# AnthonyYates/FluidFramework

Hardware: AMD Instinct MI355X
Metric: sequenced ops applied/sec (whole node) + achieved HBM GB/s, 256k docs (higher is better)
Workload: dtype int32

## Files before the change

fluidframework_amd/csrc/reg_engine.hpp:

```cpp
#pragma once
#include <stddef.h>
#include <stdint.h>
#include <string.h>

#include "engine_types.hpp"
#include "reg_rows.hpp"
#include "wave_simd.hpp"

namespace mte {

constexpr u32 RG_LEVELS = 8;
constexpr u32 RG_HEAP = 511;
constexpr u32 RSEQ_LIVE = 0x7FFFFFFFu;
constexpr u32 RCL_LIVE = 0xFFu;
constexpr i32 REG_HANDOFF = 101;
constexpr u32 NS_SHIFT = 24, NS_MASK = 3u << NS_SHIFT;

enum RgProf : u32 {
    RP_TOTAL, RP_FETCH, RP_APPLY, RP_RESOLVE, RP_INSERT_SLOT, RP_SPLIT, RP_RANGE, RP_ZAMBONI, RP_SCOUR,
    RP_HEAP, RP_FIND_SEG, RP_PACK, RP_LRU, RP_OPS, RP_N_RESOLVE, RP_N_SCOUR, RP_N_SCOUR_CHANGED,
    RP_N_PACK, RP_N_POP, RP_N_SPLIT_BLK, RP_N_MOVE, RP_SPLIT_AT, RP_INS, RP_REM, RP_MSN, RP_ZAM_EDIT,
    RP_PACK_SIBS,
    RP_PACK_FUSED,
    RP_N
};
#if defined(MTE_PROFILE) && !defined(MTE_CPU)
#ifdef RG_PROF_ONLY
#define RG_ON(slot) ((slot) == RG_PROF_ONLY || (slot) == RP_TOTAL)
#else
#define RG_ON(slot) true
#endif
template <bool ON>
struct RgScope {
    u64& acc;
    u64 t0;
    __device__ __forceinline__ RgScope(u64& a) : acc(a), t0(ON ? __builtin_amdgcn_s_memtime() : 0) {}
    __device__ __forceinline__ ~RgScope() {
        if (ON) acc += __builtin_amdgcn_s_memtime() - t0;
    }
};
#define RG_PROF(slot) RgScope<RG_ON(slot)> _rg_scope_##slot(pf[slot])
#define RG_COUNT(slot, n) (pf[slot] += (u64)(n))
#elif defined(MTE_MARKERS) && !defined(MTE_CPU)
template <u32 S>
struct RgMark {
    __device__ __forceinline__ RgMark() { asm volatile("; MTE_BEGIN %0" ::"i"(S + 100)); }
    __device__ __forceinline__ ~RgMark() { asm volatile("; MTE_END %0" ::"i"(S + 100)); }
};
#define RG_PROF(slot) RgMark<slot> _rg_mark_##slot
#define RG_COUNT(slot, n) \
    do {                  \
    } while (0)
#else
#define RG_PROF(slot) \
    do {              \
    } while (0)
#define RG_COUNT(slot, n) \
    do {                  \
    } while (0)
#endif

#if defined(MTE_CPU) && defined(MTE_CPU_STATS)
enum RgStat : u32 {
    RS_OPS, RS_RESOLVE, RS_RES_ROWS, RS_RES_NROWS, RS_POP, RS_POP_BIG, RS_POP_HEAP, RS_FIND_ROWS, RS_SCOUR,
    RS_SCOUR_NOP, RS_SCOUR_SERIAL, RS_SCOUR_COPY, RS_PACK, RS_SPLIT_BLK, RS_MOVE_SLOTS, RS_SPLIT_AT,
    RS_ZAM_CALLS, RS_ZAM_POPS, RS_LRU_PUSH, RS_RANGE_ROWS, RS_DUO_HANDOVER, RS_DUO_SPEC_OK, RS_DUO_SPEC_REDO,
    RS_DUO_NO_RESOLVE, RS_DUO_W_ROWS,
    RS_REM, RS_REM_SAMEROW, RS_REM_SAMEROW_NOSPLIT, RS_RES2_ROWS, RS_PACK_SCOUR, RS_PACK_SCOUR_NOP,
    RS_PACK_SELF_CHANGED, RS_PACK_SIB_CHANGED, RS_PACK_ONE_ROW, RS_PACK_TWO_ROWS, RS_PACK_SERIAL, RS_PACK_GC,
    RS_PACK_CASCADE, RS_PACK_M8, RS_PACK_GROWS, RS_PACK_M_SUM, RS_PACK_KK_SUM,
    RS_LRU_REWRITE, RS_LRU_FOLDED,
    RS_PACK_FUSED, RS_PACK_FUSED_FB_SERIAL, RS_PACK_FUSED_FB_GC,
    RS_HIT_FIRST, RS_HIT_SECOND, RS_SPLIT_NEXT_ROW, RS_HEAP_REG1, RS_HEAP_REG2, RS_SIFT_SERIAL, RS_PACK_KK1, RS_PACK_KK2,
    RS_PACK_KK3, RS_PACK_KK4, RS_PACK_KK5, RS_PACK_KK6, RS_PACK_KK7, RS_PACK_REM, RS_PACK_INTERNAL, RS_ROOM_REFUSED, RS_N
};
inline u64 g_rg_stats[RS_N + 64];
#define RG_STAT(i, n) (g_rg_stats[i] += (u64)(n))
struct RgDuoStat {
    u64 w;
    bool popped, packed, pending;
    void settle_begin() {
        if (pending) RG_STAT(RS_DUO_NO_RESOLVE, 1);
        w = 0;
        popped = packed = pending = false;
    }
    void settle_end() {
        if (!popped) return;
        RG_STAT(RS_DUO_HANDOVER, 1);
        RG_STAT(RS_DUO_W_ROWS, __builtin_popcountll(w));
        pending = true;
    }
    void resolved(bool ok, u32 row) {
        if (!pending) return;
        pending = false;
        const u64 scanned = ok && row < 63 ? (2ull << row) - 1 : ~0ull;
        if (packed || (w & scanned)) RG_STAT(RS_DUO_SPEC_REDO, 1);
        else RG_STAT(RS_DUO_SPEC_OK, 1);
    }
};
inline RgDuoStat g_rg_duo;
#define RG_DUO(stmt) (g_rg_duo.stmt)
#else
#define RG_STAT(i, n) \
    do {              \
    } while (0)
#define RG_DUO(stmt) \
    do {             \
    } while (0)
#endif

#ifndef MTE_FUSED_PACK
#define MTE_FUSED_PACK 1
#endif
#ifndef MTE_STATE_REGS
#define MTE_STATE_REGS 5
#endif

struct RSeg {
    u32 len;
    i32 seq;
    u32 rseq;
    u32 meta;
    u32 toff;
    u32 cap;
    u32 rm;
    u32 sid;
    u32 props = 0;
    u32 rm2 = 0;
};
struct RFound {
    bool ok;
    u32 k;
    u32 cnt;
    i32 slot;
    i32 r;
    u32 row;
    u32 carry;
};

template <int NR = (int)RG_ROWS, bool PAGED = false, bool PROPS = false, bool WIDE = false>
struct RegEngine {
    static constexpr bool kProps = PROPS, kWide = WIDE;
    static constexpr bool kFoldLru = !PAGED && NR == (int)RG_ROWS;
    static constexpr bool kFusedPack = MTE_FUSED_PACK == 2 || (MTE_FUSED_PACK == 1 && !PAGED && NR == (int)RG_ROWS);
    static constexpr bool kOwnRows = !PAGED && NR == (int)RG_ROWS && !PROPS && !WIDE;
    static constexpr bool kHeapInPlace = kOwnRows && (MTE_STATE_REGS & 1) != 0;
    static constexpr bool kMulDiv = kOwnRows && (MTE_STATE_REGS & 4) != 0;
    static constexpr u32 MAXC = WIDE ? 64u : 32u;
    typedef simd::V V;
    typedef simd::B B;
    static constexpr u32 NBLK = (u32)NR * 8;
    typedef RowStore<NR, PAGED, PROPS, WIDE> Rows;
    typedef typename Rows::Row Row;

    simd::VA<RG_LEVELS> LV;
    struct HeapRegs {
        V r0, r1, x2, x3, x4, x5, x6, x7;
        SD V get(u32 i) const {
            switch (i) {
                case 0: return r0;
                case 1: return r1;
                case 2: return x2;
                case 3: return x3;
                case 4: return x4;
                case 5: return x5;
                case 6: return x6;
                default: return x7;
            }
        }
        SD void set(u32 i, V v) {
            switch (i) {
                case 0: r0 = v; break;
                case 1: r1 = v; break;
                case 2: x2 = v; break;
                case 3: x3 = v; break;
                case 4: x4 = v; break;
                case 5: x5 = v; break;
                case 6: x6 = v; break;
                default: x7 = v; break;
            }
        }
        SD void zero() { r0 = r1 = x2 = x3 = x4 = x5 = x6 = x7 = simd::splat(0); }
    };
    HeapRegs HK, HS;
    u32 n_lb, height, heapSize, segNext, arenaTop, arenaSel;
    i32 minSeq, curSeq, heapTop, status, failSeq;
    u32 n_gc, max_lb;
    u32 n_ops, n_msgs;
    SD u32 ops_n() const { return n_ops; }
    SD u32 msgs_n() const { return n_msgs; }
    SD void set_counts(u32 o, u32 m) {
        n_ops = o;
        n_msgs = m;
    }
    SD void count_op() { n_ops++; }
    SD void count_msg() { n_msgs++; }
    u32 lb_lim;
    bool adirty;
#if defined(MTE_PROFILE) && !defined(MTE_CPU)
    u64 pf[RP_N];
#endif
    const Params& p;
    u32 doc;
    u16* payload;
    u16* arena0;
    u32 seg_cap, arena_cap, payload_len;
    Rows rows;
#ifdef MTE_CPU
    u32& pool_rows = rows.at.pool_rows;
#endif
    SD void release_rows() { rows.release_rows(); }

    SD V ld_len(u32 r) const { return rows.ldf(r, 0, 0); }
    SD V ld_meta(u32 r) const { return rows.ldf(r, 0, 3); }
    SD V ld_sid(u32 r) const { return rows.ldf(r, 1, 3); }
    SD bool ensure_blocks(u32 nb) {
        if constexpr (PAGED) {
            if (rows.grow_rows((nb + 7) >> 3)) return true;
            fail(REG_HANDOFF, curSeq);
        } else {
            if (nb <= NBLK) return true;
            fail(MTE_DOC_CAPACITY, curSeq);
        }
        return false;
    }

    SD RegEngine(const Params& p_, u32 doc_, const RowsLds& g = RowsLds::solo_lean())
        : p(p_), doc(doc_), rows(g), res_mode(g.mode) {
        setup();
    }
// ... 186 lines not shown
        f.slot = -1;
        f.r = 0;
        f.row = 0;
        f.carry = 0;
        const u32 nrows = (n_lb + 7) >> 3;
        RG_STAT(RS_RESOLVE, 1);
        RG_STAT(RS_RES_NROWS, nrows);
        u32 carry = carry0;
        const B end = (L() & 7u) == 7u;
        auto hit_row = [&](const Row& w, u32 r, u64 hit, const V& v, const V& incl) MTE_LI {
            const u32 g = (u32)__builtin_ctzll(hit) >> 3;
            const u32 k = r * 8 + g, gb = g * 8;
            const V rr = (u32)pos - (incl - v);
            const B valid = w.len != 0u;
            const B seen = simd::sle(w.rseq, R) & (w.rseq != 0u);
            const B cand = in_group(k) & valid & (simd::slt(rr, v) | ((rr == 0u) & (v == 0u) & ~seen));
            const u64 cm = simd::ballot(cand);
            f.ok = true;
            f.k = k;
            f.cnt = (u32)__builtin_popcount(group_bits(simd::ballot(valid), k));
            f.row = r;
            f.carry = carry;
            rows.cache(r, w);
            if (cm) {
                const u32 l = (u32)__builtin_ctzll(cm);
                f.slot = (i32)(l - gb);
                f.r = (i32)simd::readlane(rr, l);
            }
        };
        const u32 last = nrows - 1;
        Row a = rows.row(r0), b;
        V v, incl;
        u64 hit = 0;
        bool inb = false;
        u32 r = r0;
        for (;;) {
            b = rows.ldrow(r + 1 < last ? r + 1 : last);
            RG_COUNT(RP_N_RESOLVE, 1);
            v = vis(a, R, C);
            RG_STAT(RS_RES_ROWS, 1);
            incl = simd::scan_incl(v) + carry;
            hit = simd::ballot(end & simd::sge(incl, pos));
            if (hit) break;
            carry = simd::readlane(incl, 63);
            if (++r >= nrows) break;
            a = rows.ldrow(r + 1 < last ? r + 1 : last);
            RG_COUNT(RP_N_RESOLVE, 1);
            v = vis(b, R, C);
            RG_STAT(RS_RES_ROWS, 1);
            incl = simd::scan_incl(v) + carry;
            hit = simd::ballot(end & simd::sge(incl, pos));
            if (hit) {
                inb = true;
                break;
            }
            carry = simd::readlane(incl, 63);
            if (++r >= nrows) break;
        }
        if (!hit) {
            RG_DUO(resolved(false, 0));
            return f;
        }
        RG_STAT(inb ? RS_HIT_SECOND : RS_HIT_FIRST, nrows >= 3);
        if (inb) a = b;
        hit_row(a, r, hit, v, incl);
        RG_DUO(resolved(true, f.row));
        return f;
    }

    SD u32 parent_of(u32 lv, u32 c, u32& first) const {
        const V cnt = LV.get(lv);
        const V incl = simd::scan_incl(cnt);
        const u64 m = simd::ballot(incl > c);
        const u32 pi = m ? (u32)__builtin_ctzll(m) : 0u;
        first = simd::readlane(incl, pi) - simd::readlane(cnt, pi);
        return pi;
    }
    SD void insert_after(u32 c, u32 lv) {
        for (u32 guard = 0; guard <= RG_LEVELS; guard++) {
            if (lv + 1 >= height) {
                if (lv >= RG_LEVELS) break;
                LV.set(lv, simd::sel(L() == 0u, 2u, simd::splat(0)));
                height++;
                return;
            }
            u32 first;
            const u32 pi = parent_of(lv, c, first);
            V P = LV.get(lv);
            const u32 nc = simd::readlane(P, pi) + 1;
            if (nc < 8) {
                LV.set(lv, simd::writelane(P, pi, nc));
                return;
            }
            P = simd::sel(L() > pi, simd::wave_shr1(P), P);
            P = simd::sel((L() == pi) | (L() == pi + 1), 4u, P);
            LV.set(lv, P);
            c = pi;
            lv++;
        }
        fail(MTE_DOC_CAPACITY, curSeq);
    }

    SD void shift_blocks(u32 from, i32 d) {
        if (d == 0) return;
        RG_COUNT(RP_N_MOVE, n_lb - from);
        const u32 n = (n_lb - from) * 8;
        RG_STAT(RS_MOVE_SLOTS, n);
        if (d > 0) {
            rows.mv_slots((from + (u32)d) * 8, from * 8, n);
        } else {
            rows.mv_slots((from - (u32)(-d)) * 8, from * 8, n);
            rows.zero_slots((n_lb - (u32)(-d)) * 8, (u32)(-d) * 8);
        }
    }

    bool lruFolded = false;
    SD u32 insert_slot(u32 k, u32 cnt, u32 j, const RSeg& rec, bool upd, u32 ul, u32 uc, i32 lru = 0) {
        RG_PROF(RP_INSERT_SLOT);
        lruFolded = false;
        if (cnt >= 8 || j > cnt) {
            fail(MTE_DOC_CAPACITY, curSeq);
            return NONE;
        }
        const u32 r = k >> 3, gb = gbase(k);
        Row& w = rows.rowref(r);
        const V sl = L() & 7u;
        const B ing = in_group(k);
        const B mv = ing & (sl > j);
        const B at = L() == gb + j;
        u32 ns = (simd::readlane(w.meta, gb) >> NS_SHIFT) & 3u;
        bool push = false;
        if constexpr (kFoldLru) {
            if (lru && cnt + 1 < 8) {
                lruFolded = true;
                if (ns != SC_TRUE && lru > curSeq) {
                    push = true;
                    ns = SC_TRUE;
                    ns_put(w, k, SC_TRUE);
                }
            }
        }
        if (upd) {
            const B lf = L() == gb + j - 1;
            w.len = simd::sel(lf, ul, w.len);
            w.cap = simd::sel(lf, uc, w.cap);
        }
        auto put = [&](V& x, u32 val) MTE_LI {
            x = simd::sel(mv, simd::row_shr1(x), x);
            x = simd::sel(at, val, x);
        };
        put(w.len, rec.len);
        put(w.seq, (u32)rec.seq);
        put(w.rseq, rec.rseq);
        put(w.meta, (rec.meta & ~NS_MASK) | (ns << NS_SHIFT));
        put(w.toff, rec.toff);
        put(w.cap, rec.cap);
        put(w.rm, rec.rm);
        put(w.sid, rec.sid);
        if constexpr (PROPS) put(w.props, rec.props);
        if constexpr (WIDE) put(w.rm2, rec.rm2);
        rows.writeback(r);
        if (push) {
            RG_STAT(RS_LRU_FOLDED, 1);
            heap_push(rec.sid, lru);
        }
        if (cnt + 1 < 8) return k;
        split_block(k);
        return j < 4 ? k : k + 1;
    }
    SD void split_block(u32 k) {
        RG_PROF(RP_SPLIT);
        RG_COUNT(RP_N_SPLIT_BLK, 1);
        RG_STAT(RS_SPLIT_BLK, 1);
        if (!ensure_blocks(n_lb + 1)) return;
        shift_blocks(k + 1, 1);
        const u32 r = k >> 3, r2 = (k + 1) >> 3;
        RG_STAT(RS_SPLIT_NEXT_ROW, r2 != r);
        const V sl = L() & 7u;
        const B lo = in_group(k + 1) & (sl < 4u), hi2 = in_group(k + 1) & (sl >= 4u), hi = in_group(k) & (sl >= 4u);
        const V src = (L() + (r2 == r ? 0u : 64u) - 4u) & 63u;
        Row w = rows.row(r);
        const u32 nsk = simd::readlane(w.meta, gbase(k)) & NS_MASK;
        Row w2 = r2 == r ? w : rows.ldrow(r2);
        auto mv = [&](V& x, V& y, u32 keepHi) MTE_LI {
            const V moved = simd::bperm(x, src);
            if (r2 == r) {
                x = simd::sel(lo, moved, x);
                x = simd::sel(hi2, 0u, x);
                x = simd::sel(hi, keepHi, x);
            } else {
                y = simd::sel(lo, moved, simd::sel(hi2, 0u, y));
                x = simd::sel(hi, keepHi, x);
            }
        };
        mv(w.len, w2.len, 0u);
        mv(w.seq, w2.seq, 0u);
        mv(w.rseq, w2.rseq, 0u);
        mv(w.meta, w2.meta, nsk);
        mv(w.toff, w2.toff, 0u);
        mv(w.cap, w2.cap, 0u);
        mv(w.rm, w2.rm, 0u);
        mv(w.sid, w2.sid, 0u);
        if constexpr (PROPS) mv(w.props, w2.props, 0u);
        if constexpr (WIDE) mv(w.rm2, w2.rm2, 0u);
        if (r2 == r) {
            w.meta = simd::sel(in_group(k + 1), w.meta & ~NS_MASK, w.meta);
            rows.putrow(r, w);
        } else {
            w2.meta = simd::sel(in_group(k + 1), w2.meta & ~NS_MASK, w2.meta);
            rows.strow(r2, w2);
            rows.putrow(r, w);
        }
        n_lb++;
        if (n_lb > max_lb) max_lb = n_lb;
        insert_after(k, 0);
    }

    template <int D>
    SD static u32 hrd(const HeapRegs& A, u32 q) {
        const u32 l = q & 63u;
        if constexpr (D <= 5) {
            return simd::readlane(A.get(0), l);
        } else if constexpr (D == 6) {
            return simd::readlane(A.get(1), l);
        } else if constexpr (D == 7) {
            const u32 a = simd::readlane(A.get(2), l), b = simd::readlane(A.get(3), l);
            return (q >> 6) & 1u ? b : a;
        } else {
            const u32 a = simd::readlane(A.get(4), l), b = simd::readlane(A.get(5), l);
            const u32 c = simd::readlane(A.get(6), l), d = simd::readlane(A.get(7), l);
            const u32 r = (q >> 6) & 3u;
            return r == 0 ? a : r == 1 ? b : r == 2 ? c : d;
        }
    }
    template <int D>
    SD static void hwr(HeapRegs& A, u32 q, u32 v) {
        [[maybe_unused]] const u32 l = q & 63u;
        if constexpr (kHeapInPlace && D >= 7) {
            if constexpr (D == 7) {
                A.x2 = simd::sel(L() == q - 128u, v, A.x2);
                A.x3 = simd::sel(L() == q - 192u, v, A.x3);
            } else {
                A.x4 = simd::sel(L() == q - 256u, v, A.x4);
                A.x5 = simd::sel(L() == q - 320u, v, A.x5);
                A.x6 = simd::sel(L() == q - 384u, v, A.x6);
                A.x7 = simd::sel(L() == q - 448u, v, A.x7);
            }
        } else if constexpr (D <= 5) {
            A.set(0, simd::writelane(A.get(0), l, v));
        } else if constexpr (D == 6) {
            A.set(1, simd::writelane(A.get(1), l, v));
// ... 875 lines not shown
    }

    SD void zamboni() {
        RG_PROF(RP_ZAMBONI);
        RG_STAT(RS_ZAM_CALLS, 1);
        for (int i = 0; i < 2 && !status; i++) {
            if (heapSize == 0 || heapTop > minSeq) break;
            RG_STAT(RS_ZAM_POPS, 1);
            const u32 k = heap_pop_find();
            if (k == NONE) continue;
            if (ns_get(k) == SC_FALSE) continue;
            const u32 cnt = count(k);
            const u32 nc = scour(k, cnt);
            if (status) return;
            if (!scoured) ns_set(k, SC_FALSE);
            if (!(nc < cnt && nc < 4 && height > 1)) continue;
            u32 k0;
            const u32 pi = parent_of(0, k, k0);
            const u32 m = simd::readlane(LV.get(0), pi);
            if (m == 0 || m > 8 || k0 + m > n_lb) {
                fail(MTE_DOC_CAPACITY, curSeq);
                return;
            }
            V cn = simd::splat(0);
#if defined(MTE_CPU) && defined(MTE_CPU_STATS)
            const u64 serial0 = g_rg_stats[RS_SCOUR_SERIAL];
            const u32 gc0 = n_gc;
            RG_STAT(((k0 + m - 1) >> 3) == (k0 >> 3) ? RS_PACK_ONE_ROW : RS_PACK_TWO_ROWS, 1);
            RG_STAT(RS_PACK_M8, m == 8);
            RG_STAT(RS_PACK_M_SUM, m);
#endif
            if constexpr (kFusedPack) {
                if (pack_fused(pi, m, k0, k)) continue;
            }
            {
                RG_PROF(RP_PACK_SIBS);
                for (u32 idx = 0; idx < m; idx++) {
                    RG_STAT(RS_PACK_SCOUR, 1);
                    const u32 c = scour(k0 + idx, count(k0 + idx));
                    if (status) return;
                    if (!scoured) RG_STAT(RS_PACK_SCOUR_NOP, 1);
                    else RG_STAT(k0 + idx == k ? RS_PACK_SELF_CHANGED : RS_PACK_SIB_CHANGED, 1);
                    cn = simd::writelane(cn, idx, c);
                }
            }
#if defined(MTE_CPU) && defined(MTE_CPU_STATS)
            RG_STAT(RS_PACK_SERIAL, g_rg_stats[RS_SCOUR_SERIAL] != serial0);
            RG_STAT(RS_PACK_GC, n_gc != gc0);
#endif
            pack_leaves(pi, m, k0, cn);
        }
    }

    SD u32 split_at(const RFound& f) {
        RG_PROF(RP_SPLIT_AT);
        RG_STAT(RS_SPLIT_AT, 1);
        const u32 r = f.k >> 3, l = gbase(f.k) + (u32)f.slot;
        const Row w = rows.row(r);
        RSeg t;
        t.len = simd::readlane(w.len, l);
        t.seq = (i32)simd::readlane(w.seq, l);
        t.rseq = simd::readlane(w.rseq, l);
        t.meta = simd::readlane(w.meta, l);
        t.toff = simd::readlane(w.toff, l);
        t.cap = simd::readlane(w.cap, l);
        t.rm = simd::readlane(w.rm, l);
        if constexpr (PROPS) t.props = simd::readlane(w.props, l);
        if constexpr (WIDE) t.rm2 = simd::readlane(w.rm2, l);
        const u32 sid = new_sid();
        if (sid == NONE) return NONE;
        const u32 rr = (u32)f.r;
        const bool ar = (t.toff & ARENA_BIT) != 0;
        const u32 lc = ar ? rr : 0u;
        RSeg right = t;
        right.len = t.len - rr;
        right.toff = t.toff + rr;
        right.cap = ar ? t.cap - rr : 0u;
        right.sid = sid;
        return insert_slot(f.k, f.cnt, (u32)f.slot + 1, right, true, rr, lc);
    }

    SD bool op_insert(i32 pos, i32 R, u32 C, i32 seq, RSeg rec) {
        RG_PROF(RP_INS);
        RFound f = resolve(pos, R, C);
        if (!f.ok) {
            fail(MTE_DOC_INSERT_FAILED, seq);
            return false;
        }
        u32 k = f.k, j;
        if (f.slot >= 0 && f.r > 0) {
            if (split_at(f) == NONE || status) return false;
            const u32 s = (u32)f.slot;
            if (f.cnt + 1 < 8 || s + 1 < 4) {
                j = s + 1;
                f.cnt = f.cnt + 1 < 8 ? f.cnt + 1 : 4;
            } else if (s == 3) {
                j = 4;
                f.cnt = 4;
            } else {
                k = f.k + 1;
                j = s - 3;
                f.cnt = 4;
            }
        } else {
            j = f.slot >= 0 ? (u32)f.slot : f.cnt;
        }
        if (rec.len == 0) return false;
        rec.sid = new_sid();
        if (rec.sid == NONE) return false;
        const u32 b = insert_slot(k, f.cnt, j, rec, false, 0, 0, seq > minSeq ? seq : 0);
        if (status) return false;
        if (seq > minSeq && !lruFolded) add_lru(b, rec.sid, seq);
        return status == 0;
    }

    SD bool op_remove(i32 p1, i32 p2, i32 R, u32 C, i32 seq) {
        RG_PROF(RP_REM);
        u32 r1 = 0, c1 = 0;
        RG_STAT(RS_REM, 1);
        [[maybe_unused]] bool f1ok = false, bsplit = false;
        for (u32 ph = 0; ph < 2; ph++) {
            const RFound f = resolve(ph ? p2 : p1, R, C, r1, c1);
            if (ph == 0 && f.ok) {
                r1 = f.row;
                c1 = f.carry;
                f1ok = true;
            }
            const bool split = f.ok && f.slot >= 0 && f.r > 0;
            bsplit = bsplit || (split && f.cnt + 1 >= 8);
            if (ph) {
                RG_STAT(RS_RES2_ROWS, f.ok ? f.row - r1 + 1 : ((n_lb + 7) >> 3) - r1);
                RG_STAT(RS_REM_SAMEROW, f1ok && f.ok && f.row == r1);
                RG_STAT(RS_REM_SAMEROW_NOSPLIT, f1ok && f.ok && f.row == r1 && !bsplit);
            }
            if (!split) continue;
            if (split_at(f) == NONE || status) return false;
        }
        RG_PROF(RP_RANGE);
        const u32 nrows = (n_lb + 7) >> 3;
        u32 carry = c1;
        const u32 cbit = WIDE ? 1u << (C & 31u) : 1u << C;
        for (u32 r = r1; r < nrows && (i32)carry < p2; r++) {
            RG_STAT(RS_RANGE_ROWS, 1);
            Row& w = rows.rowref(r);
            const V v = vis(w, R, C);
            const V incl = simd::scan_incl(v) + carry;
            const V ex = incl - v;
            const B mark = (v != 0u) & simd::slt(ex, p2) & simd::sgt(incl, p1);
            carry = simd::readlane(incl, 63);
            const u64 mm = simd::ballot(mark);
            if (!mm) continue;
            const B was = mark & (w.rseq != RSEQ_LIVE);
            const B fresh = simd::andn(mark, was);
            if (WIDE && C >= 32) {
                if constexpr (WIDE) w.rm2 = simd::sel(mark, w.rm2 | cbit, w.rm2);
            } else {
                w.rm = simd::sel(mark, w.rm | cbit, w.rm);
            }
            w.meta = simd::sel(was, w.meta | F_OVL, simd::sel(fresh, (w.meta & ~0xFF00u) | (C << 8) | F_REMOVED, w.meta));
            w.rseq = simd::sel(fresh, (u32)seq, w.rseq);
            if constexpr (kFoldLru) {
                u64 pm = 0;
                if (seq > curSeq) {
                    const u64 nst = simd::ballot(((w.meta >> NS_SHIFT) & 3u) == SC_TRUE);
                    u64 grp = 0;
                    for (u64 gm = mm & ~nst; gm;) {
                        const u32 l = (u32)__builtin_ctzll(gm);
                        const u64 g8 = 0xFFull << (l & ~7u);
                        gm &= ~g8;
                        pm |= 1ull << l;
                        grp |= g8;
                    }
                    if (grp) w.meta = simd::sel(simd::ballot_mask(grp), (w.meta & ~NS_MASK) | (SC_TRUE << NS_SHIFT), w.meta);
                }
                rows.writeback(r);
                for (; pm; pm &= pm - 1) {
                    RG_STAT(RS_LRU_FOLDED, 1);
                    heap_push(simd::readlane(w.sid, (u32)__builtin_ctzll(pm)), seq);
                    if (status) return false;
                }
            } else {
                rows.writeback(r);
                for (u64 gm = mm; gm;) {
                    const u32 l = (u32)__builtin_ctzll(gm);
                    const u32 g = l >> 3;
                    gm &= ~(0xFFull << (g * 8));
                    add_lru(r * 8 + g, simd::readlane(w.sid, l), seq);
                    if (status) return false;
                }
            }
        }
        return status == 0;
    }

    SD bool op_annotate(i32 p1, i32 p2, i32 R, u32 C, i32 seq, u32 propset, bool rewrite) {
        RG_PROF(RP_REM);
        u32 r1 = 0, c1 = 0;
        for (u32 ph = 0; ph < 2; ph++) {
            const RFound f = resolve(ph ? p2 : p1, R, C, r1, c1);
            if (ph == 0 && f.ok) {
                r1 = f.row;
                c1 = f.carry;
            }
            if (!f.ok || !(f.slot >= 0 && f.r > 0)) continue;
            if (split_at(f) == NONE || status) return false;
        }
        RG_PROF(RP_RANGE);
        const u32 nrows = (n_lb + 7) >> 3;
        u32 carry = c1, memoOld = NONE, memoNew = 0;
        for (u32 r = r1; r < nrows && (i32)carry < p2; r++) {
            Row& w = rows.rowref(r);
            const V v = vis(w, R, C);
            const V incl = simd::scan_incl(v) + carry;
            const V ex = incl - v;
            const B mark = (v != 0u) & simd::slt(ex, p2) & simd::sgt(incl, p1);
            carry = simd::readlane(incl, 63);
            const u64 mm = simd::ballot(mark);
            if (!mm) continue;
            for (u64 pending = mm; pending;) {
                const u32 old = simd::readlane(w.props, (u32)__builtin_ctzll(pending));
                u32 nid;
                if (old == memoOld) {
                    nid = memoNew;
                } else {
                    nid = build_map(old, propset, rewrite);
                    if (status) return false;
                    memoOld = old;
                    memoNew = nid;
                }
                const B same = simd::ballot_mask(pending) & (w.props == old);
                w.props = simd::sel(same, nid, w.props);
                pending &= ~simd::ballot(same);
            }
            rows.writeback(r);
            for (u64 gm = mm; gm;) {
                const u32 l = (u32)__builtin_ctzll(gm);
                const u32 g = l >> 3;
                gm &= ~(0xFFull << (g * 8));
                add_lru(r * 8 + g, simd::readlane(w.sid, l), seq);
                if (status) return false;
            }
        }
        return status == 0;
    }

    SD bool room() {
        if constexpr (PAGED) {
            const u32 keep = (n_lb + 7) >> 3;
            if (rows.n_rows > keep) rows.shrink_rows(keep);
            return n_lb + 4 <= lb_lim && heapSize + n_lb + 8 < RG_HEAP && height + 2 <= RG_LEVELS &&
                   (n_lb < 57 || simd::readlane(LV.get(0), 56) == 0u);
        }
        return n_lb + 16 <= lb_lim && heapSize + n_lb + 8 < RG_HEAP && height + 2 <= RG_LEVELS &&
               (n_lb < 57 || simd::readlane(LV.get(0), 56) == 0u);
    }

    SD bool apply(const mte_op& op) {
        RG_PROF(RP_APPLY);
        bool edited = false;
        if (!apply_edit(op, edited)) return false;
        if (status) return true;
        RG_DUO(settle_begin());
        apply_settle(op.seq, op.msn, (op.flags & MTE_F_END_OF_MSG) != 0, edited);
        RG_DUO(settle_end());
        return true;
    }
    SD bool apply_edit(const mte_op& op, bool& edited) {
        RG_STAT(RS_OPS, 1);
        const u32 type = op.type;
        const bool ins = type == MTE_OP_INSERT || type == MTE_OP_INSERT_MARKER;
        const bool ann = PROPS && type == MTE_OP_ANNOTATE;
        if (!(ins || ann || type == MTE_OP_REMOVE || type == MTE_OP_NOOP)) return false;
        if ((op.flags & (MTE_F_REL | MTE_F_PERM)) || (!PROPS && op.props)) return false;
        if (type != MTE_OP_NOOP && (op.client == 0 || op.client >= MAXC)) return false;
        if (!room()) {
            RG_STAT(RS_ROOM_REFUSED, 1);
            return false;
        }
        const u32 C = op.client;
// ... 397 lines not shown
```

fluidframework_amd/csrc/reg_rows.hpp:

```cpp
#pragma once
#include <stddef.h>
#include <stdint.h>
#include <string.h>

#include "engine_types.hpp"
#include "wave_simd.hpp"

namespace mte {

constexpr u32 RG_ROWS = 32;
constexpr u32 RG_BLOCKS = RG_ROWS * 8;
constexpr u32 ROWS_POOL_WORDS = 3;
constexpr u32 ROWS_WAIT_TRIES = 20000;
static_assert(RG_BLOCKS <= SOLO_POOL, "the rows live in the SoloPlan's slot arrays");
static_assert(RG_ROWS <= CK_MAX_ROWS, "checkpoint regions hold the whole row plan");

template <bool P, bool W>
struct RowProps {};
template <>
struct RowProps<true, false> {
    simd::V props;
};
template <>
struct RowProps<false, true> {
// ... 81 lines not shown
};

#ifndef MTE_CPU
extern __shared__ uint4 g_lds_dyn[];

template <bool PAGED, bool PROPS, bool WIDE>
struct RowMem : RowTable<RowsLds, PAGED, PROPS, WIDE> {
    typedef RowTable<RowsLds, PAGED, PROPS, WIDE> T;
    typedef simd::V V;
    typedef simd::B B;
    typedef typename T::Row Row;
    using T::at;
    using T::cr;
    using T::prow;
    using T::ptab;
    SD explicit RowMem(const RowsLds& g) : T(g) {}
    template <class X>
    SD static X* lds(u32 off) { return reinterpret_cast<X*>(reinterpret_cast<unsigned char*>(g_lds_dyn) + off); }
    SD uint4* VISP() const { return lds<uint4>(at.vis); }
    SD uint4* AUXP() const { return lds<uint4>(at.aux); }
    SD u32* PROPP() const { return lds<u32>(at.props); }
    SD u32* RM2P() const { return lds<u32>(at.rm2); }
    SD u32* pool_words() const { return lds<u32>(at.mask); }
    SD bool take_row(u32& row) {
        u32 got = NONE;
        if (__lane_id() == 0) {
            u32* m = pool_words();
            for (u32 wd = 0; wd < ROWS_POOL_WORDS && got == NONE; wd++) {
                u32 cur = __hip_atomic_load(m + wd, __ATOMIC_RELAXED, __HIP_MEMORY_SCOPE_WORKGROUP);
                while (~cur) {
                    const u32 bit = 1u << __builtin_ctz(~cur);
                    const u32 old = atomicOr(m + wd, bit);
                    if (!(old & bit)) {
                        got = wd * 32 + (u32)__builtin_ctz(bit);
                        break;
                    }
                    cur = old | bit;
                }
            }
        }
        got = simd::readlane(simd::V{got}, 0);
        row = got;
        return got != NONE;
    }
    SD bool claim_row(u32& row) {
        for (u32 t = 0; t < ROWS_WAIT_TRIES; t++) {
            if (take_row(row)) return true;
            __builtin_amdgcn_s_sleep(8);
        }
        return take_row(row);
    }
    SD void give_row(u32 row) {
        if (__lane_id() == 0) atomicAnd(pool_words() + (row >> 5), ~(1u << (row & 31)));
    }
    SD void zero_prow(u32 row) {
        VISP()[row * 64 + __lane_id()] = make_uint4(0, 0, 0, 0);
        AUXP()[row * 64 + __lane_id()] = make_uint4(0, 0, 0, 0);
        if constexpr (PROPS) PROPP()[row * 64 + __lane_id()] = 0u;
        if constexpr (WIDE) RM2P()[row * 64 + __lane_id()] = 0u;
        simd::lds_order();
    }
    SD u32 pslot(u32 s) const {
        if constexpr (PAGED) return simd::bperm(ptab, simd::V{s >> 6}).x * 64u + (s & 63u);
        else return s;
    }
    SD Row ldrow(u32 r) const {
        const u32 i = prow(r) * 64 + __lane_id();
        const uint4 v = VISP()[i], a = AUXP()[i];
        Row w;
        w.len = V{v.x}, w.seq = V{v.y}, w.rseq = V{v.z}, w.meta = V{v.w};
        w.cap = V{a.x}, w.toff = V{a.y}, w.rm = V{a.z}, w.sid = V{a.w};
        if constexpr (PROPS) w.props = V{PROPP()[i]};
        if constexpr (WIDE) w.rm2 = V{RM2P()[i]};
        return w;
    }
    SD void strow(u32 r, const Row& w) {
        const u32 i = prow(r) * 64 + __lane_id();
        VISP()[i] = make_uint4(w.len.x, w.seq.x, w.rseq.x, w.meta.x);
        AUXP()[i] = make_uint4(w.cap.x, w.toff.x, w.rm.x, w.sid.x);
        if constexpr (PROPS) PROPP()[i] = w.props.x;
        if constexpr (WIDE) RM2P()[i] = w.rm2.x;
        simd::lds_order();
    }
    SD V ldf(u32 r, u32 aux, u32 c) const {
        const u32* b = reinterpret_cast<const u32*>(aux ? AUXP() : VISP());
        return V{b[(prow(r) * 64 + __lane_id()) * 4 + c]};
    }
    SD void stf(u32 r, u32 aux, u32 c, V x, B m) {
        u32* b = reinterpret_cast<u32*>(aux ? AUXP() : VISP());
        if (simd::lane_of(m)) b[(prow(r) * 64 + __lane_id()) * 4 + c] = x.x;
        simd::lds_order();
    }
    SD void mv_slots(u32 dst, u32 src, u32 n) {
        cr = NONE;
        uint4* V4 = VISP();
        uint4* A4 = AUXP();
        const u32 L = __lane_id();
        if constexpr (PAGED) {
            const bool up = dst > src;
            for (u32 c = 0; c < n; c += 64) {
                const i32 i = up ? (i32)(n - c) - 64 + (i32)L : (i32)(c + L);
                const bool ok = i >= 0 && (u32)i < n;
                const u32 ii = ok ? (u32)i : 0u;
                const u32 ps = pslot(src + ii), pd = pslot(dst + ii);
                uint4 v = make_uint4(0, 0, 0, 0), a = v;
                u32 pp = 0, q2 = 0;
                if (ok) {
                    v = V4[ps];
                    a = A4[ps];
                    if constexpr (PROPS) pp = PROPP()[ps];
                    if constexpr (WIDE) q2 = RM2P()[ps];
                }
                simd::lds_order();
                if (ok) {
                    V4[pd] = v;
                    A4[pd] = a;
                    if constexpr (PROPS) PROPP()[pd] = pp;
                    if constexpr (WIDE) RM2P()[pd] = q2;
                }
                simd::lds_order();
            }
            return;
        }
        if constexpr (!PROPS && !WIDE) {
            const uint4 z = make_uint4(0, 0, 0, 0);
            if (dst > src) {
                i32 i = (i32)n - 64 + (i32)L;
                uint4 v = z, a = z;
                if (i >= 0) {
                    v = V4[src + (u32)i];
                    a = A4[src + (u32)i];
                }
                for (i32 b = (i32)n - 64; b > -64; b -= 64) {
                    const i32 j = i - 64;
                    uint4 v2 = z, a2 = z;
                    if (b - 64 > -64 && j >= 0) {
                        v2 = V4[src + (u32)j];
                        a2 = A4[src + (u32)j];
                    }
                    simd::lds_order();
                    if (i >= 0) {
                        V4[dst + (u32)i] = v;
                        A4[dst + (u32)i] = a;
                    }
                    simd::lds_order();
                    v = v2;
                    a = a2;
                    i = j;
                }
            } else {
                u32 i = L;
                uint4 v = z, a = z;
                if (i < n) {
                    v = V4[src + i];
                    a = A4[src + i];
                }
                for (u32 b = 0; b < n; b += 64) {
                    const u32 j = i + 64;
                    uint4 v2 = z, a2 = z;
                    if (b + 64 < n && j < n) {
                        v2 = V4[src + j];
                        a2 = A4[src + j];
                    }
                    simd::lds_order();
                    if (i < n) {
                        V4[dst + i] = v;
// ... 37 lines not shown
                    a = A4[src + i];
                    if constexpr (PROPS) pp = PROPP()[src + i];
                    if constexpr (WIDE) q2 = RM2P()[src + i];
                }
                simd::lds_order();
                if (i < n) {
                    V4[dst + i] = v;
                    A4[dst + i] = a;
                    if constexpr (PROPS) PROPP()[dst + i] = pp;
                    if constexpr (WIDE) RM2P()[dst + i] = q2;
                }
                simd::lds_order();
            }
        }
    }
    SD void zero_slots(u32 s0, u32 n) {
        cr = NONE;
        if constexpr (!PAGED && !PROPS && !WIDE) {
            for (u32 b = __lane_id(); b < n; b += 64) {
                VISP()[s0 + b] = make_uint4(0, 0, 0, 0);
                AUXP()[s0 + b] = make_uint4(0, 0, 0, 0);
            }
            simd::lds_order();
            return;
        }
        for (u32 c = 0; c < n; c += 64) {
            const u32 b = c + __lane_id();
            const u32 ps = pslot(s0 + (b < n ? b : 0u));
            if (b < n) {
                VISP()[ps] = make_uint4(0, 0, 0, 0);
                AUXP()[ps] = make_uint4(0, 0, 0, 0);
                if constexpr (PROPS) PROPP()[ps] = 0u;
                if constexpr (WIDE) RM2P()[ps] = 0u;
            }
        }
        simd::lds_order();
    }
};

#else
struct RowArrays {
    u32 mem[ROW_FIELDS_MAX][RG_ROWS * 64];
    u64 pool_mask = 0;
    u32 pool_rows = RG_ROWS, pool_takes = 0;
    explicit RowArrays(const RowsLds&) {}
};
template <bool PAGED, bool PROPS, bool WIDE>
struct RowMem : RowTable<RowArrays, PAGED, PROPS, WIDE> {
    typedef RowTable<RowArrays, PAGED, PROPS, WIDE> T;
    typedef simd::V V;
    typedef simd::B B;
    typedef typename T::Row Row;
    using T::at;
    using T::cr;
    using T::prow;
    explicit RowMem(const RowsLds& g) : T(g) {}
    SD u32 pslot(u32 s) const { return PAGED ? prow(s >> 6) * 64 + (s & 63) : s; }
    SD bool claim_row(u32& row) {
        for (u32 t = 0; t < at.pool_rows; t++) {
            const u32 c = (at.pool_takes * 7 + 3 + t) % at.pool_rows;
            if (!((at.pool_mask >> c) & 1)) {
                at.pool_mask |= 1ull << c;
                at.pool_takes++;
                row = c;
                return true;
            }
        }
        return false;
    }
    SD void give_row(u32 row) { at.pool_mask &= ~(1ull << row); }
    SD void zero_prow(u32 row) {
        for (auto& f : at.mem) memset(&f[row * 64], 0, 64 * 4);
    }
    SD Row ldrow(u32 r) const {
        Row w;
        const u32 pr = prow(r);
        w.for_each_field([&](u32 id, V& x) { memcpy(x.x, &at.mem[id][pr * 64], 64 * 4); });
        return w;
    }
    SD void strow(u32 r, const Row& w) {
        const u32 pr = prow(r);
        w.for_each_field([&](u32 id, const V& x) { memcpy(&at.mem[id][pr * 64], x.x, 64 * 4); });
    }
    SD V ldf(u32 r, u32 aux, u32 c) const {
        V x;
        memcpy(x.x, &at.mem[aux * 4 + c][prow(r) * 64], 64 * 4);
        return x;
    }
    SD void stf(u32 r, u32 aux, u32 c, V x, B m) {
        const u32 pr = prow(r);
        for (u32 l = 0; l < 64; l++)
            if ((m.m >> l) & 1) at.mem[aux * 4 + c][pr * 64 + l] = x.x[l];
    }
    SD void mv_slots(u32 dst, u32 src, u32 n) {
        cr = NONE;
        for (auto& f : at.mem) {
            if (!PAGED) {
                memmove(&f[dst], &f[src], (size_t)n * 4);
                continue;
            }
            for (u32 t = 0; t < n; t++) {
                const u32 i = dst > src ? n - 1 - t : t;
                f[pslot(dst + i)] = f[pslot(src + i)];
            }
        }
    }
    SD void zero_slots(u32 s0, u32 n) {
        cr = NONE;
        for (auto& f : at.mem)
            for (u32 i = 0; i < n; i++) f[pslot(s0 + i)] = 0;
    }
};
#endif

template <int NR, bool PAGED, bool PROPS, bool WIDE>
struct RowStore : RowMem<PAGED, PROPS, WIDE> {
    typedef RowMem<PAGED, PROPS, WIDE> M;
    typedef typename M::Row Row;
    using M::cr;
    using M::cw;
    using M::ldrow;
    using M::n_rows;
    using M::pool_full;
    using M::ptab;
    using M::strow;
    SD explicit RowStore(const RowsLds& g) : M(g) {}
    SD Row row(u32 r) {
        if (r != cr) {
            cw = ldrow(r);
            cr = r;
        }
        return cw;
    }
    SD void putrow(u32 r, const Row& w) {
        strow(r, w);
        cw = w;
        cr = r;
    }
    SD Row& rowref(u32 r) {
        if (r != cr) {
            cw = ldrow(r);
            cr = r;
        }
        return cw;
    }
    SD void writeback(u32 r) { strow(r, cw); }
    SD void cache(u32 r, const Row& w) {
        cw = w;
        cr = r;
    }
    SD void drop_row() { cr = NONE; }

    SD void reset_rows() {
        n_rows = 0;
        ptab = simd::splat(0);
    }
    SD bool grow_rows(u32 need) {
        while (n_rows < need) {
            u32 row;
            if (n_rows >= (u32)NR) return false;
            if (!M::claim_row(row)) {
                pool_full = true;
                return false;
            }
            M::zero_prow(row);
            ptab = simd::writelane(ptab, n_rows, row);
            n_rows++;
        }
        return true;
    }
    SD void shrink_rows(u32 keep) {
        cr = NONE;
        while (n_rows > keep) M::give_row(M::prow(--n_rows));
    }
    SD void release_rows() {
        if constexpr (PAGED) shrink_rows(0);
    }
    SD bool rows_whole(u32 n_lb) const {
        if constexpr (PAGED) return n_rows * 8 >= n_lb;
        else return true;
    }
};

}
```

Before: 84.37 million.

## Fuse block split into insert_slot using register permutes on the cached row

```diff
diff --git a/fluidframework_amd/csrc/reg_engine.hpp b/fluidframework_amd/csrc/reg_engine.hpp
--- a/fluidframework_amd/csrc/reg_engine.hpp
+++ b/fluidframework_amd/csrc/reg_engine.hpp
@@ -72,7 +72,13 @@
     RS_LRU_REWRITE, RS_LRU_FOLDED,
     RS_PACK_FUSED, RS_PACK_FUSED_FB_SERIAL, RS_PACK_FUSED_FB_GC,
     RS_HIT_FIRST, RS_HIT_SECOND, RS_SPLIT_NEXT_ROW, RS_HEAP_REG1, RS_HEAP_REG2, RS_SIFT_SERIAL, RS_PACK_KK1, RS_PACK_KK2,
-    RS_PACK_KK3, RS_PACK_KK4, RS_PACK_KK5, RS_PACK_KK6, RS_PACK_KK7, RS_PACK_REM, RS_PACK_INTERNAL, RS_ROOM_REFUSED, RS_N
+    RS_PACK_KK3, RS_PACK_KK4, RS_PACK_KK5, RS_PACK_KK6, RS_PACK_KK7, RS_PACK_REM, RS_PACK_INTERNAL, RS_ROOM_REFUSED,
+    RS_SPLIT_FUSED, RS_SPLIT_UPD, RS_SPLIT_INS, RS_SPLIT_REM, RS_SPLIT_J0, RS_SPLIT_J1, RS_SPLIT_J2, RS_SPLIT_J3,
+    RS_SPLIT_J4, RS_SPLIT_J5, RS_SPLIT_J6, RS_SPLIT_J7, RS_SPLIT_G0, RS_SPLIT_G1, RS_SPLIT_G2, RS_SPLIT_G3, RS_SPLIT_G4,
+    RS_SPLIT_G5, RS_SPLIT_G6, RS_SPLIT_G7, RS_SPLIT_NEW_ROW, RS_SPLIT_FIRST, RS_SPLIT_LAST, RS_SPLIT_ROWS_AFTER0,
+    RS_SPLIT_ROWS_AFTER1, RS_SPLIT_ROWS_AFTER2, RS_SPLIT_ROWS_AFTER3P, RS_SPLIT_TAIL_ROW, RS_SPLIT_TAIL_LATER,
+    RS_SPLIT_CASCADE, RS_SPLIT_ROOT, RS_SPLIT_LRU_DUE, RS_SPLIT_LRU_MARKS, RS_SPLIT_NS_SET, RS_SPLIT_UPD_THEN_INS,
+    RS_SPLIT_TWICE, RS_REM_SPLIT2_ONE_ROW, RS_REM_SPLIT2_TWO_ROWS, RS_SPLIT_REFUSED, RS_N
 };
 inline u64 g_rg_stats[RS_N + 64];
 #define RG_STAT(i, n) (g_rg_stats[i] += (u64)(n))
@@ -100,6 +106,15 @@
 };
 inline RgDuoStat g_rg_duo;
 #define RG_DUO(stmt) (g_rg_duo.stmt)
+struct RgSplitCtx {
+    bool in_rem = false, upd_split = false, parent_split = false, root_grew = false;
+    u32 rem_splits = 0, rem_row = 0, lb0 = 0;
+};
+inline RgSplitCtx g_rg_split;
+#define RG_CTX(...)  \
+    do {             \
+        __VA_ARGS__; \
+    } while (0)
 #else
 #define RG_STAT(i, n) \
     do {              \
@@ -107,6 +122,9 @@
 #define RG_DUO(stmt) \
     do {             \
     } while (0)
+#define RG_CTX(...) \
+    do {            \
+    } while (0)
 #endif
 
 #ifndef MTE_FUSED_PACK
@@ -114,6 +132,9 @@
 #endif
 #ifndef MTE_STATE_REGS
 #define MTE_STATE_REGS 5
+#endif
+#ifndef MTE_FUSED_SPLIT
+#define MTE_FUSED_SPLIT 1
 #endif
 
 struct RSeg {
@@ -146,6 +167,7 @@
     static constexpr bool kOwnRows = !PAGED && NR == (int)RG_ROWS && !PROPS && !WIDE;
     static constexpr bool kHeapInPlace = kOwnRows && (MTE_STATE_REGS & 1) != 0;
     static constexpr bool kMulDiv = kOwnRows && (MTE_STATE_REGS & 4) != 0;
+    static constexpr bool kFusedSplit = MTE_FUSED_SPLIT == 2 || (MTE_FUSED_SPLIT == 1 && kOwnRows);
     static constexpr u32 MAXC = WIDE ? 64u : 32u;
     typedef simd::V V;
     typedef simd::B B;
@@ -498,6 +520,7 @@
                 if (lv >= RG_LEVELS) break;
                 LV.set(lv, simd::sel(L() == 0u, 2u, simd::splat(0)));
                 height++;
+                RG_CTX(g_rg_split.root_grew = true);
                 return;
             }
             u32 first;
@@ -508,6 +531,7 @@
                 LV.set(lv, simd::writelane(P, pi, nc));
                 return;
             }
+            RG_CTX(g_rg_split.parent_split = true);
             P = simd::sel(L() > pi, simd::wave_shr1(P), P);
             P = simd::sel((L() == pi) | (L() == pi + 1), 4u, P);
             LV.set(lv, P);
@@ -560,6 +584,61 @@
             const B lf = L() == gb + j - 1;
             w.len = simd::sel(lf, ul, w.len);
             w.cap = simd::sel(lf, uc, w.cap);
+        }
+        RG_CTX(if (cnt + 1 == 8) split_stat(k, j, upd, lru, ns));
+        if constexpr (kFusedSplit) {
+            if (cnt + 1 == 8 && ensure_blocks(n_lb + 1)) {
+                RG_PROF(RP_SPLIT);
+                RG_COUNT(RP_N_SPLIT_BLK, 1);
+                RG_COUNT(RP_N_MOVE, n_lb - (k + 1));
+                RG_STAT(RS_SPLIT_BLK, 1);
+                RG_STAT(RS_SPLIT_FUSED, 1);
+                RG_STAT(RS_MOVE_SLOTS, (n_lb - (k + 1)) * 8);
+                const u32 g = k & 7u;
+                RG_STAT(RS_SPLIT_NEXT_ROW, g == 7u);
+                const u32 nsk = ns << NS_SHIFT;
+                const u32 rmeta = rec.meta & ~NS_MASK;
+                const V grp = L() >> 3;
+                const B gk = grp == g, gn = grp == ((g + 1u) & 7u);
+                Row y;
+                {
+                    const V tt = sl + simd::sel(gn, 4u, simd::splat(0));
+                    const V d = simd::sel(simd::andn(grp > g, gn), 8u, simd::sel(gn, 4u, simd::splat(0)) + simd::sel((gk | gn) & (tt > j), 1u, simd::splat(0)));
+                    const V src = (L() - d) & 63u;
+                    const B rat = L() == ((gb + j + (j >= 4u ? 4u : 0u)) & 63u);
+                    const B emp = (gk | gn) & (sl >= 4u);
+                    auto fs = [&](V& o, const V& x, u32 val) MTE_LI { o = simd::sel(emp, 0u, simd::sel(rat, val, simd::bperm(x, src))); };
+                    fs(y.meta, w.meta, rmeta | nsk);
+                    y.meta = simd::sel(gk & (sl >= 4u), nsk, simd::sel(gn, y.meta & ~NS_MASK, y.meta));
+                    fs(y.len, w.len, rec.len);
+                    fs(y.seq, w.seq, (u32)rec.seq);
+                    fs(y.rseq, w.rseq, rec.rseq);
+                    fs(y.toff, w.toff, rec.toff);
+                    fs(y.cap, w.cap, rec.cap);
+                    fs(y.rm, w.rm, rec.rm);
+                    fs(y.sid, w.sid, rec.sid);
+                    if constexpr (PROPS) fs(y.props, w.props, rec.props);
+                    if constexpr (WIDE) fs(y.rm2, w.rm2, rec.rm2);
+                }
+                if (g == 7u) {
+                    auto back = [&](V& x, const V& o) MTE_LI { x = simd::sel(gn, x, o); };
+                    back(w.len, y.len), back(w.seq, y.seq), back(w.rseq, y.rseq), back(w.meta, y.meta);
+                    back(w.toff, y.toff), back(w.cap, y.cap), back(w.rm, y.rm), back(w.sid, y.sid);
+                    if constexpr (PROPS) back(w.props, y.props);
+                    if constexpr (WIDE) back(w.rm2, y.rm2);
+                } else {
+                    w = y;
+                }
+                const u32 from = r * 8 + (g < 7u ? 7u : 8u);
+                if (n_lb > from) rows.mv_later((from + 1) * 8, from * 8, (n_lb - from) * 8);
+                if (g == 7u) rows.strow_lanes(r + 1, y, L() < 8u);
+                rows.writeback(r);
+                n_lb++;
+                if (n_lb > max_lb) max_lb = n_lb;
+                insert_after(k, 0);
+                RG_CTX(split_stat_end());
+                return j < 4 ? k : k + 1;
+            }
         }
         auto put = [&](V& x, u32 val) MTE_LI {
             x = simd::sel(mv, simd::row_shr1(x), x);
@@ -581,8 +660,45 @@
             heap_push(rec.sid, lru);
         }
         if (cnt + 1 < 8) return k;
-        split_block(k);
+        if constexpr (kFusedSplit) {
+            RG_COUNT(RP_N_SPLIT_BLK, 1);
+            RG_STAT(RS_SPLIT_BLK, 1);
+        } else {
+            split_block(k);
+        }
+        RG_CTX(split_stat_end());
         return j < 4 ? k : k + 1;
+    }
+    SD void split_stat([[maybe_unused]] u32 k, [[maybe_unused]] u32 j, [[maybe_unused]] bool upd, [[maybe_unused]] i32 lru,
+                       [[maybe_unused]] u32 ns) {
+        RG_STAT(upd ? RS_SPLIT_UPD : RS_SPLIT_INS, 1);
+        RG_STAT(RS_SPLIT_J0 + j, 1);
+        RG_STAT(RS_SPLIT_G0 + (k & 7u), 1);
+        RG_STAT(RS_SPLIT_NEW_ROW, (k & 7u) == 7u && k + 1 == n_lb);
+        RG_STAT(RS_SPLIT_FIRST, k == 0);
+        RG_STAT(RS_SPLIT_LAST, k + 1 == n_lb);
+        [[maybe_unused]] const u32 lastrow = (n_lb - 1) >> 3, ra = lastrow - (k >> 3);
+        RG_STAT(ra >= 3 ? RS_SPLIT_ROWS_AFTER3P : RS_SPLIT_ROWS_AFTER0 + ra, 1);
+        [[maybe_unused]] const u32 rowend = ((k >> 3) + 1) * 8 < n_lb ? ((k >> 3) + 1) * 8 : n_lb;
+        RG_STAT(RS_SPLIT_TAIL_ROW, rowend - (k + 1));
+        RG_STAT(RS_SPLIT_TAIL_LATER, n_lb - rowend);
+        RG_STAT(RS_SPLIT_LRU_DUE, lru != 0 && lru > curSeq);
+        RG_STAT(RS_SPLIT_LRU_MARKS, lru != 0 && lru > curSeq && ns != SC_TRUE);
+        RG_STAT(RS_SPLIT_NS_SET, ns == SC_TRUE);
+        RG_CTX(if (upd && g_rg_split.in_rem) {
+            RG_STAT(RS_SPLIT_REM, 1);
+            if (g_rg_split.rem_splits++ == 0) g_rg_split.rem_row = k >> 3;
+            else RG_STAT((k >> 3) == g_rg_split.rem_row ? RS_REM_SPLIT2_ONE_ROW : RS_REM_SPLIT2_TWO_ROWS, 1);
+        });
+        RG_CTX(if (!upd && g_rg_split.upd_split) RG_STAT(RS_SPLIT_TWICE, 1));
+        RG_CTX(if (upd && !g_rg_split.in_rem) g_rg_split.upd_split = true);
+        RG_CTX(g_rg_split.parent_split = g_rg_split.root_grew = false);
+        RG_CTX(g_rg_split.lb0 = n_lb);
+    }
+    SD void split_stat_end() {
+        RG_CTX(RG_STAT(RS_SPLIT_CASCADE, g_rg_split.parent_split));
+        RG_CTX(RG_STAT(RS_SPLIT_ROOT, g_rg_split.root_grew));
+        RG_CTX(RG_STAT(RS_SPLIT_REFUSED, n_lb == g_rg_split.lb0));
     }
     SD void split_block(u32 k) {
         RG_PROF(RP_SPLIT);
@@ -1624,6 +1740,7 @@
 
     SD bool op_insert(i32 pos, i32 R, u32 C, i32 seq, RSeg rec) {
         RG_PROF(RP_INS);
+        RG_CTX(g_rg_split = RgSplitCtx());
         RFound f = resolve(pos, R, C);
         if (!f.ok) {
             fail(MTE_DOC_INSERT_FAILED, seq);
@@ -1650,6 +1767,7 @@
         if (rec.len == 0) return false;
         rec.sid = new_sid();
         if (rec.sid == NONE) return false;
+        RG_CTX(if (g_rg_split.upd_split) RG_STAT(RS_SPLIT_UPD_THEN_INS, 1));
         const u32 b = insert_slot(k, f.cnt, j, rec, false, 0, 0, seq > minSeq ? seq : 0);
         if (status) return false;
         if (seq > minSeq && !lruFolded) add_lru(b, rec.sid, seq);
@@ -1660,6 +1778,7 @@
         RG_PROF(RP_REM);
         u32 r1 = 0, c1 = 0;
         RG_STAT(RS_REM, 1);
+        RG_CTX(g_rg_split = RgSplitCtx(); g_rg_split.in_rem = true);
         [[maybe_unused]] bool f1ok = false, bsplit = false;
         for (u32 ph = 0; ph < 2; ph++) {
             const RFound f = resolve(ph ? p2 : p1, R, C, r1, c1);
@@ -1737,6 +1856,7 @@
 
     SD bool op_annotate(i32 p1, i32 p2, i32 R, u32 C, i32 seq, u32 propset, bool rewrite) {
         RG_PROF(RP_REM);
+        RG_CTX(g_rg_split = RgSplitCtx());
         u32 r1 = 0, c1 = 0;
         for (u32 ph = 0; ph < 2; ph++) {
             const RFound f = resolve(ph ? p2 : p1, R, C, r1, c1);
diff --git a/fluidframework_amd/csrc/reg_rows.hpp b/fluidframework_amd/csrc/reg_rows.hpp
--- a/fluidframework_amd/csrc/reg_rows.hpp
+++ b/fluidframework_amd/csrc/reg_rows.hpp
@@ -187,6 +187,16 @@
         if constexpr (WIDE) RM2P()[i] = w.rm2.x;
         simd::lds_order();
     }
+    SD void strow_lanes(u32 r, const Row& w, B m) {
+        const u32 i = prow(r) * 64 + __lane_id();
+        if (simd::lane_of(m)) {
+            VISP()[i] = make_uint4(w.len.x, w.seq.x, w.rseq.x, w.meta.x);
+            AUXP()[i] = make_uint4(w.cap.x, w.toff.x, w.rm.x, w.sid.x);
+            if constexpr (PROPS) PROPP()[i] = w.props.x;
+            if constexpr (WIDE) RM2P()[i] = w.rm2.x;
+        }
+        simd::lds_order();
+    }
     SD V ldf(u32 r, u32 aux, u32 c) const {
         const u32* b = reinterpret_cast<const u32*>(aux ? AUXP() : VISP());
         return V{b[(prow(r) * 64 + __lane_id()) * 4 + c]};
@@ -390,6 +400,13 @@
         const u32 pr = prow(r);
         w.for_each_field([&](u32 id, const V& x) { memcpy(&at.mem[id][pr * 64], x.x, 64 * 4); });
     }
+    SD void strow_lanes(u32 r, const Row& w, B m) {
+        const u32 pr = prow(r);
+        w.for_each_field([&](u32 id, const V& x) {
+            for (u32 l = 0; l < 64; l++)
+                if ((m.m >> l) & 1) at.mem[id][pr * 64 + l] = x.x[l];
+        });
+    }
     SD V ldf(u32 r, u32 aux, u32 c) const {
         V x;
         memcpy(x.x, &at.mem[aux * 4 + c][prow(r) * 64], 64 * 4);
@@ -458,6 +475,11 @@
         cr = r;
     }
     SD void drop_row() { cr = NONE; }
+    SD void mv_later(u32 dst, u32 src, u32 n) {
+        const u32 c = cr;
+        M::mv_slots(dst, src, n);
+        cr = c;
+    }
 
     SD void reset_rows() {
         n_rows = 0;
```

Result: slower. 82.70 million (-2.0%).
